# bchess/k8s-1m

Hardware: AMD Instinct MI355X
Metric: pods scheduled/sec at 1M nodes (1/2/4/8 GPU) + % of HBM roofline (higher is better)
Workload: dtype int64+f64

## Files before the change

### k8s-1m_amd/csrc/ksched_host.cpp

```cpp
#include <atomic>
#include <hip/hip_runtime.h>
#include <rccl/rccl.h>

#include <algorithm>
#include <array>
#include <chrono>
#include <cstdarg>
#include <cstdio>
#include <cstdlib>
#include <condition_variable>
#include <cstring>
#include <deque>
#include <functional>
#include <map>
#include <mutex>
#include <set>
#include <thread>
#include <memory>
#include <string>
#include <unordered_map>
#include <unordered_set>
#include <vector>

#include "ksched.h"
// ... 246 lines not shown
  uint32_t dict_version = 0;
  uint32_t names_version = 0;
  bool ext = false, norm = false;
  uint32_t cap_pods = 0;
  size_t cap_words = 0;
  PodDev *d_pods = nullptr;
  double *d_pinv = nullptr;
  uint64_t *d_clauses = nullptr;
  DevResult *d_results = nullptr;
  DevResult *h_results = nullptr;
  PodDev *h_pods = nullptr;
  double *h_pinv = nullptr;
  uint64_t *h_clauses = nullptr;
  size_t n_words = 0;
  bool uploaded = false;
  std::vector<uint32_t> set_ids;
  std::vector<uint8_t> spread;
  bool any_spread = false;
  std::vector<SoloNeeds> solo;
  std::vector<uint64_t> ports;
  std::vector<uint8_t> rep;
  std::vector<uint32_t> class_refs;
  std::vector<uint32_t> term_refs;
  uint64_t *d_cmask = nullptr, *h_cmask = nullptr;
  uint8_t *d_marks = nullptr;
  uint32_t *d_cls = nullptr, *h_cls = nullptr;
  bool dups = false;
  bool ran = false;
  ForgetBits forgotten;
  bool queued = false, done = false;
  ks_status run_status = KS_OK;
  std::string run_err;
};

struct LgPost {
  hipEvent_t ev = nullptr;
  const void *ptr = nullptr;
  std::vector<double> vals;
};
struct LocalGroup : Rendezvous<LgPost> {
  using Post = LgPost;
  explicit LocalGroup(uint32_t n) : Rendezvous<LgPost>(n) {}
};

struct ks_ctx {
  ks_config cfg{};
  std::string err;
  hipStream_t stream = nullptr;
  hipStream_t rstream = nullptr;
  hipStream_t sstream = nullptr;
  hipEvent_t ev_sw[2] = {nullptr, nullptr}, ev_res[2] = {nullptr, nullptr};
  hipEvent_t ev_swept[2] = {nullptr, nullptr}, ev_fixed[2] = {nullptr, nullptr};
  uint32_t *d_flags = nullptr;
  uint32_t round_seq = 0;
  uint32_t seq_of[2] = {0, 0};
  bool value_sync = true;
  uint32_t sync_timeout_ms = 60000;
  std::atomic<bool> wedged{false};
  hipStream_t diag_stream = nullptr;
  uint32_t flag_want[4] = {0, 0, 0, 0};
  uint32_t *h_diag = nullptr;
  int32_t stall_flag = -1;
  uint32_t stall_us = 0;
  ks_fit_strategy fit{KS_FIT_LEAST_ALLOCATED, 1, 1, 0};
  FitParams fit_params{0, 1, 1, fit_weight_rcp(1), fit_weight_rcp(1), fit_weight_rcp(2)};
  uint32_t fit_general = 0;
  std::vector<ks_fit_shape_point> fit_shape;
  std::vector<std::pair<uint32_t, int32_t>> fit_x;
  std::vector<std::string> fit_x_names;
  std::vector<int64_t> ba_list;
  std::vector<std::string> ba_names;
  bool early_fix = true;
  uint32_t resolve_mode = KS_RESOLVE_AUTO;
  uint32_t par_max_passes = 32, serial_rounds = 4;
  bool res_profile = false;
  bool dedup = true;
  bool tuple_guess = true;
  uint32_t timing_every = 8, ext_npl = 2;
  uint32_t sweep_blocks = 4096, sweep_blocks_ext = 16384;
  uint64_t sweep_geom[2][8] = {};
  bool ev_profile = false;
  bool run_profile = false;
  double prof[PROF_SLOTS] = {};
  struct EvProf {
    uint64_t runs = 0, events = 0;
    double s = 0;
  } ev_prof[4];
  uint32_t cap = 0, S = 1, npl = 8, P = 256, K = 256;
  std::vector<Shard> shards;
  uint32_t npos = 0;
  std::vector<uint32_t> slot_pos;
  NodeTable t{};
  NodeTable run_t{};
  Shard *d_shards = nullptr;
  uint32_t *d_slot_pos = nullptr;
  uint32_t *d_start = nullptr;
  uint32_t *h_start = nullptr;
  uint32_t *d_norm = nullptr;
  double *d_norm_inv = nullptr;
  PodStat *d_pstat = nullptr;
  uint32_t *d_fix = nullptr;
  uint32_t *d_dedup = nullptr;
  bool dedup_used[2] = {false, false};
  BlockRec *d_brec = nullptr;
  size_t brec_bytes = 0;
  uint64_t *d_srec = nullptr, *d_frec = nullptr;
// ... 2404 lines not shown
  a.slot_pos = c->d_slot_pos;
  a.w = Weights{c->cfg.weight_fit, c->cfg.weight_balanced, c->cfg.weight_taint, c->cfg.weight_affinity,
                c->cfg.weight_image};
  a.fs = c->fit_params;
  a.fit_general = c->fit_general;
  a.fit_table = c->d_fit_table;
  if ((size_t)nloc * c->P * bmax * sizeof(BlockRec) > c->brec_bytes)
    return c->fail(KS_ERR_INVALID, "block record buffer too small");

  const bool early = b->norm && !multi && c->early_fix;
  a.pstat_sweep = early ? 1u : 0u;
  if (k >= 2) {
    if ((st = hand_wait(c, c->stream, 2, c->ev_res[q], c->seq_of[q]))) return st;
    if (b->norm && !early && (st = hand_wait(c, c->stream, 3, c->ev_fixed[pq], c->seq_of[pq]))) return st;
    HIPC(c, launch_advance_writeback(a, c->d_carry + (size_t)q * MAX_P, c->d_pipe + 4 + q, c->stream));
  } else {
    HIPC(c, launch_advance(a, c->stream));
  }
  hipEvent_t e0 = nullptr, e1 = nullptr;
  if (tm) {
    e0 = get_event(c);
    e1 = get_event(c);
    HIPC(c, hipEventRecord(e0, c->stream));
  }
  if (early) HIPC(c, hipMemsetAsync(c->d_pstat, 0, (size_t)c->P * sizeof(PodStat), c->stream));
  HIPC(c, launch_sweep(a, b->ext, bmax, groups, nloc, c->stream));
  ++c->sweeps_issued;
  {
    uint64_t *g = c->sweep_geom[b->ext ? 1 : 0];
    ++g[0];
    g[1] = knpl;
    g[2] = b->ext ? sweep_label_words(knpl, a.t.lw) : 0;
    g[3] = sub;
    g[4] = bmax;
    g[5] = groups;
    g[6] = pg;
  }
  if (tm) {
    HIPC(c, hipEventRecord(e1, c->stream));
    c->ev_sweep.emplace_back(e0, e1);
  }
  const uint32_t seq = ++c->round_seq;
  c->seq_of[q] = seq;
  hipStream_t ss = c->sstream;
  if (early) {
    HIPC(c, launch_norm_check(a, c->stream));
    RoundArgs f = a;
    f.fix = 1;
    f.pg = MAX_PG;
    HIPC(c, launch_sweep(f, true, bmax, (c->P + MAX_PG - 1) / MAX_PG, nloc, c->stream));
  }
  if ((st = hand_signal(c, c->stream, 0, c->ev_swept[q], seq)) || (st = hand_wait(c, ss, 0, c->ev_swept[q], seq))) return st;
  if (b->norm && !early) HIPC(c, hipMemsetAsync(c->d_pstat, 0, (size_t)c->P * sizeof(PodStat), ss));
  HIPC(c, launch_merge(a, nloc, ss));
  if (b->norm && !early) {
    if (multi && (st = coll_allreduce_max_u32(c, (uint32_t *)c->d_pstat, 4 * (size_t)c->P, ss))) return st;
    HIPC(c, launch_norm_check(a, ss));
    RoundArgs f = a;
    f.fix = 1;
    f.pg = MAX_PG;
    HIPC(c, launch_sweep(f, true, bmax, (c->P + MAX_PG - 1) / MAX_PG, nloc, ss));
    if ((st = hand_signal(c, ss, 3, c->ev_fixed[q], seq))) return st;
    HIPC(c, launch_merge(f, nloc, ss));
  }
  if (multi) {
    const size_t words = (size_t)c->P * RW;
    if ((st = coll_allgather(c, a.srec, words * 8, ss))) return st;
  }
  if (c->S > 1) HIPC(c, launch_merge_shards(a, ss));
  HIPC(c, launch_gather_cand(a, b->ext, ss));
  if (k > 0) {
    if ((st = hand_wait(c, ss, 2, c->ev_res[pq], seq - 1))) return st;
    HIPC(c, launch_patch(a, b->ext, ss));
  }
  if ((st = hand_signal(c, ss, 1, c->ev_sw[q], seq)) || (st = hand_wait(c, c->rstream, 1, c->ev_sw[q], seq))) return st;
  if (tm) {
    e0 = get_event(c);
    e1 = get_event(c);
    HIPC(c, hipEventRecord(e0, c->rstream));
  }
  {
    RoundArgs ra = a;
    ra.flag_res = c->value_sync ? c->d_flags + 2 : nullptr;
    ra.seq = seq;
    ra.stall_us = 0;
    if (c->stall_flag == 2) {
      ra.stall_us = c->stall_us;
      c->stall_flag = -1;
    }
    c->flag_want[2] = seq;
    ra.par_max_passes = c->par_max_passes;
    ra.prof = c->res_profile ? c->d_counters + 16 : nullptr;
    ra.serial_rounds = c->serial_rounds;
    ra.rmode = c->resolve_mode == KS_RESOLVE_AUTO ? c->d_flags + 4 : nullptr;
    ra.serial_only = c->resolve_mode == KS_RESOLVE_SERIAL ? 1u : 0u;
    HIPC(c, launch_resolve(ra, b->ext, c->rstream));
  }
  if (tm) {
    HIPC(c, hipEventRecord(e1, c->rstream));
    c->ev_resolve.emplace_back(e0, e1);
  }
  HIPC(c, hipEventRecord(c->ev_res[q], c->rstream));
  return KS_OK;
}

ks_status drain_rounds(ks_ctx *c, uint32_t rounds, void *h_res, const void *d_res, size_t res_bytes) {
  for (uint32_t k = rounds >= 2 ? rounds - 2 : 0; k < rounds; ++k) {
    const uint32_t q = k & 1u;
    HIPC(c, hipStreamWaitEvent(c->stream, c->ev_res[q], 0));
    HIPC(c, launch_writeback(c->t, c->d_carry + (size_t)q * MAX_P, c->d_pipe + 4 + q, c->stream));
  }
  if (res_bytes) HIPC(c, hipMemcpyAsync(h_res, d_res, res_bytes, hipMemcpyDeviceToHost, c->stream));
  HIPC(c, hipMemcpyAsync(c->h_start, c->d_start, 4, hipMemcpyDeviceToHost, c->stream));
  return sync_bounded(c, c->stream, "a pipeline run's drain");
}


ks_status batch_acquire(ks_ctx *c, uint32_t n, size_t words, ks_batch **out) {
  const uint32_t need = std::max<uint32_t>(n, 1);
  ks_batch *b = nullptr;
  {
    std::lock_guard<std::mutex> g(c->pool_mu);
    size_t bi = SIZE_MAX;
    for (size_t i = 0; i < c->pool.size(); ++i)
      if (c->pool[i]->cap_pods >= need && (bi == SIZE_MAX || c->pool[i]->cap_pods < c->pool[bi]->cap_pods)) bi = i;
    if (bi != SIZE_MAX) {
      b = c->pool[bi];
      c->pool.erase(c->pool.begin() + (long)bi);
// ... 2551 lines not shown
```

### k8s-1m_amd/csrc/ksched_kernels.hip

```cpp
#include <hip/hip_runtime.h>

#include <utility>

#include "ksched_dev.hpp"
#include "ksched_eval.hpp"
#include "ksched_kernels.hpp"
#include "ksched_instr.hpp"
#include "ksched_util.hpp"

namespace ks {




typedef unsigned u32x4 __attribute__((ext_vector_type(4)));
typedef const __attribute__((address_space(4))) u32x4 *const_words;
__device__ __forceinline__ PodDev load_pod_requests(const PodDev *pods, uint32_t i) {
  static_assert(offsetof(PodDev, req_cpu_d) == 32 && offsetof(PodDev, nz100_cpu) == 48 &&
                offsetof(PodDev, tol_hard) == 64, "PodDev: the binary64 request fields");
  const const_words src = (const_words)(pods + i);
  const u32x4 w2 = src[2], w3 = src[3];
  PodDev p = {};
  __builtin_memcpy(&p.req_cpu_d, &w2, 16);
  __builtin_memcpy(&p.nz100_cpu, &w3, 16);
// ... 508 lines not shown
  __syncthreads();
  if (threadIdx.x % WAVE == 0) scratch[wid] = v;
  __syncthreads();
  uint32_t s = 0;
  for (uint32_t i = 0; i < nw; ++i) s += scratch[i];
  __syncthreads();
  return s;
}

__device__ void merge_lists(const uint64_t *keys, size_t list_stride, const uint64_t *bounds,
                            size_t bound_stride, uint32_t nl, uint32_t len, uint32_t K, uint64_t *out,
                            uint64_t *s_sort, uint64_t *s_scr, uint32_t *s_cnt, uint32_t *s_u32) {
  uint64_t b = 0;
  for (uint32_t i = threadIdx.x; i < nl; i += blockDim.x) b = max(b, bounds[i * bound_stride]);
  b = block_max_u64(b, s_scr);
  uint32_t cnt = 0;
  for (uint32_t i = threadIdx.x; i < nl; i += blockDim.x)
    for (uint32_t q = 0; q < len; ++q) cnt += keys[i * list_stride + q] > b;
  cnt = block_sum_u32(cnt, s_u32);
  if (cnt > MERGE_CAP) {
    const uint32_t c = MERGE_CAP / nl;
    uint64_t b2 = b;
    for (uint32_t i = threadIdx.x; i < nl; i += blockDim.x)
      if (c < len) b2 = max(b2, keys[i * list_stride + c]);
    b = block_max_u64(b2, s_scr);
  }
  if (threadIdx.x == 0) *s_cnt = 0;
  __syncthreads();
  for (uint32_t i = threadIdx.x; i < nl; i += blockDim.x)
    for (uint32_t q = 0; q < len; ++q) {
      const uint64_t k = keys[i * list_stride + q];
      if (k > b) {
        const uint32_t at = atomicAdd(s_cnt, 1u);
        if (at < MERGE_CAP) s_sort[at] = k;
      }
    }
  __syncthreads();
  const uint32_t n = min(*s_cnt, (uint32_t)MERGE_CAP);
  uint32_t m = 64;
  while (m < n) m <<= 1;
  for (uint32_t i = n + threadIdx.x; i < m; i += blockDim.x) s_sort[i] = 0;
  __syncthreads();
  bitonic_desc(s_sort, m);
  const uint32_t keep = min(n, K);
  if (n > K) b = max(b, s_sort[K]);
  for (uint32_t i = threadIdx.x; i < K; i += blockDim.x) out[REC_HDR_WORDS + i] = i < keep ? s_sort[i] : 0ull;
  if (threadIdx.x == 0) {
    out[0] = b;
    ((uint32_t *)out)[2] = keep;
  }
}

constexpr int MERGE_THREADS = 1024;
__global__ __launch_bounds__(MERGE_THREADS) void merge_kernel(RoundArgs a) {
  __shared__ uint64_t s_sort[MERGE_CAP];
  __shared__ uint64_t s_scr[16];
  __shared__ uint32_t s_u32[16];
  __shared__ uint32_t s_cnt;
  __shared__ uint32_t s_wc[MERGE_THREADS / WAVE][NFILT + 5];
  const uint32_t start = uniform_u32(*a.sstart);
  const uint32_t r = blockIdx.x;
  if (start + r >= a.npods || r >= a.P) return;
  if (a.fix && a.fix_flag[r] == 0) return;
  if (a.rep != nullptr && a.rep[r] != r) return;
  const uint32_t sh = blockIdx.y;
  const Shard s = a.shards[a.shard0 + sh];
  const uint32_t nb = (s.waves * a.sub + 3) / 4;
  const BlockRec *br = a.brec + ((size_t)sh * a.P + r) * a.bstride;
  uint64_t *out = a.srec + ((size_t)(a.shard0 + sh) * a.P + r) * rec_words(a.K);
  merge_lists(&br[0].keys[0], sizeof(BlockRec) / 8, &br[0].bound, sizeof(BlockRec) / 8, nb, BLOCK_KEYS, a.K,
              out, s_sort, s_scr, &s_cnt, s_u32);
  int32_t c[NFILT + 3];
  for (int q = 0; q < NFILT + 3; ++q) c[q] = 0;
  uint32_t tmx = 0, nmx = 0;
  for (uint32_t i = threadIdx.x; i < nb; i += blockDim.x) {
    c[0] += br[i].feasible;
    for (int q = 0; q < NFILT; ++q) c[1 + q] += br[i].fails[q];
    c[6] += br[i].tt_cnt;
    c[7] += br[i].na_cnt;
    tmx = max(tmx, br[i].tt_max);
    nmx = max(nmx, br[i].na_max);
  }
  const uint32_t wid = threadIdx.x / WAVE;
#pragma unroll
  for (int q = 0; q < NFILT + 3; ++q) c[q] = wave_sum_i32_dpp(c[q]);
  tmx = wave_max_u32_dpp(tmx);
  nmx = wave_max_u32_dpp(nmx);
  if (threadIdx.x % WAVE == 0) {
    for (int q = 0; q < NFILT + 3; ++q) s_wc[wid][q] = (uint32_t)c[q];
    s_wc[wid][NFILT + 3] = tmx;
    s_wc[wid][NFILT + 4] = nmx;
  }
  __syncthreads();
  if (threadIdx.x == 0) {
    uint32_t t[NFILT + 5] = {};
    for (uint32_t w = 0; w < blockDim.x / WAVE; ++w) {
      for (int q = 0; q < NFILT + 3; ++q) t[q] += s_wc[w][q];
      t[NFILT + 3] = max(t[NFILT + 3], s_wc[w][NFILT + 3]);
      t[NFILT + 4] = max(t[NFILT + 4], s_wc[w][NFILT + 4]);
    }
    ShardRecHdr *h = (ShardRecHdr *)out;
    h->feasible = t[0];
    for (int q = 0; q < NFILT; ++q) h->fails[q] = t[1 + q];
    h->tt_cnt = t[6];
    h->na_cnt = t[7];
    if (a.pstat != nullptr && !a.fix && !a.pstat_sweep) {
      PodStat *ps = a.pstat + r;
      if (t[NFILT + 3]) atomicMax(&ps->tt_max, t[NFILT + 3]);
      if (t[NFILT + 4]) atomicMax(&ps->na_max, t[NFILT + 4]);
      if (t[0]) atomicMax(&ps->any_feasible, 1u);
    }
  }
}


__global__ __launch_bounds__(MAX_P) void norm_check_kernel(RoundArgs a) {
  __shared__ uint32_t s_wn[MAX_P / WAVE];
  const uint32_t start = uniform_u32(*a.sstart);
  const uint32_t r = threadIdx.x;
  bool wrong = false, listed = false;
  if (r < a.P && start + r < a.npods) {
    const PodDev &p = a.pods[start + r];
    const uint32_t rr = a.rep != nullptr ? a.rep[r] : r;
    PodStat st = a.pstat[rr];
    if (a.pstat_sweep) {
      st.any_feasible = st.tt_max != 0u;
      st.tt_max = st.tt_max ? st.tt_max - 1u : 0u;
      st.na_max = st.na_max ? st.na_max - 1u : 0u;
    }
    uint32_t tt = p.tt_guess, na = p.na_guess;
    if (st.any_feasible) {
      wrong = ((p.flags & PF_TT) && st.tt_max != tt) || ((p.flags & PF_NA) && st.na_max != na);
      tt = st.tt_max;
      na = st.na_max;
    }
    a.norm_max[2 * r] = tt;
    a.norm_max[2 * r + 1] = na;
    a.norm_inv[2 * r] = tt ? 1.0 / (double)tt : 0.0;
    a.norm_inv[2 * r + 1] = na ? 1.0 / (double)na : 0.0;
    a.fix_flag[r] = wrong ? 1u : 0u;
    if (wrong) mark_pod(a.marks, start + r, MARK_FIX);
    listed = wrong && rr == r;
  }
  const uint64_t wb = __ballot(listed);
  const uint32_t nw = (uint32_t)__popcll(wb), nwrong = (uint32_t)__popcll(__ballot(wrong));
  const uint32_t wid = threadIdx.x / WAVE, lane = threadIdx.x % WAVE;
  if (lane == 0) s_wn[wid] = nw;
  if (nwrong && lane == 0) atomicAdd((unsigned long long *)&a.counters[4], (unsigned long long)nwrong);
  __syncthreads();
  uint32_t idx = (uint32_t)__popcll(wb & ((1ull << lane) - 1ull)), total = 0;
#pragma unroll
  for (int w = 0; w < MAX_P / WAVE; ++w) {
    idx += (uint32_t)w < wid ? s_wn[w] : 0u;
    total += s_wn[w];
  }
  if (listed) a.fix_list[idx] = r;
  if (r >= total) a.fix_list[r] = FIX_NONE;
  if (r < MAX_P / MAX_PG) a.fix_group[r] = r * MAX_PG < total ? 1u : 0u;
}

__global__ __launch_bounds__(256) void merge_shards_kernel(RoundArgs a) {
  __shared__ uint64_t s_sort[MERGE_CAP];
  __shared__ uint64_t s_scr[16];
  __shared__ uint32_t s_u32[16];
  __shared__ uint32_t s_cnt;
  const uint32_t start = uniform_u32(*a.sstart);
  const uint32_t r = blockIdx.x;
  if (start + r >= a.npods || r >= a.P) return;
  if (a.rep != nullptr && a.rep[r] != r) return;
  const uint32_t W = rec_words(a.K);
  const uint64_t *in = a.srec + (size_t)r * W;
  const size_t stride = (size_t)a.P * W;
  uint64_t *out = a.frec + (size_t)r * W;
  merge_lists(in + REC_HDR_WORDS, stride, in, stride, a.total_shards, a.K, a.K, out, s_sort, s_scr, &s_cnt, s_u32);
  if (threadIdx.x == 0) {
    ShardRecHdr *h = (ShardRecHdr *)out;
    uint32_t f = 0, ttc = 0, nac = 0, fl[NFILT] = {0, 0, 0, 0, 0};
    for (uint32_t q = 0; q < a.total_shards; ++q) {
      const ShardRecHdr *x = (const ShardRecHdr *)(in + q * stride);
      f += x->feasible;
      ttc += x->tt_cnt;
      nac += x->na_cnt;
      for (int z = 0; z < NFILT; ++z) fl[z] += x->fails[z];
    }
    h->feasible = f;
    h->tt_cnt = ttc;
    h->na_cnt = nac;
    for (int z = 0; z < NFILT; ++z) h->fails[z] = fl[z];
  }
}

__device__ __forceinline__ CandRow cand_row(int64_t acpu, int64_t amem, int64_t rc, int64_t rm, int64_t zc, int64_t zm,
                                            int32_t apods, int32_t np, uint32_t pos) {
  CandRow w;
  w.acpu = (double)acpu;
  w.amem = (double)amem;
  w.inv_cpu = acpu ? 1.0 / w.acpu : 0.0;
  w.inv_mem = amem ? 1.0 / w.amem : 0.0;
  w.rc = (double)rc;
  w.rm = (double)rm;
  w.zc100 = (double)zc * 100.0;
  w.zm100 = (double)zm * 100.0;
  w.apods = apods;
  w.np = np;
  w.pos = pos;
  w._pad = 0;
  return w;
}

template <bool EXT>
__global__ __launch_bounds__(256) void gather_cand_kernel(RoundArgs a) {
  const uint32_t start = uniform_u32(*a.sstart);
  const uint32_t r = blockIdx.x;
  if (start + r >= a.npods || r >= a.P) return;
  if (a.rep != nullptr && a.rep[r] != r) return;
  const uint64_t *rec = a.frec + (size_t)r * rec_words(a.K);
  const uint32_t nk = ((const ShardRecHdr *)rec)->nkeys;
  for (uint32_t t = threadIdx.x; t < nk; t += blockDim.x) {
    const uint64_t k = rec[REC_HDR_WORDS + t];
    const uint32_t pos = a.slot_pos[0xFFFFFFFFu - (uint32_t)k];
    a.crow[(size_t)r * a.K + t] = cand_row(a.t.acpu[pos], a.t.amem[pos], a.t.rcpu[pos], a.t.rmem[pos], a.t.zcpu[pos],
                                           a.t.zmem[pos], a.t.apods[pos], a.t.npods[pos], pos);
    if (EXT) {
      CandExt x;
      x.w[0] = a.t.hard[pos];
      x.w[1] = a.t.prefer[pos];
#pragma unroll
      for (int q = 0; q < LW; ++q) x.w[2 + q] = a.t.lab[(size_t)q * a.t.npos + pos];
#pragma unroll
      for (int q = 0; q < NNUM; ++q) x.w[2 + LW + q] = (uint64_t)a.t.num[(size_t)q * a.t.npos + pos];
      a.cext[(size_t)r * a.K + t] = x;
    }
  }
}

constexpr int PHASH = 1024;
static_assert(2 * MAX_P >= MAX_K, "patch thread counts");


__device__ __forceinline__ uint32_t count_greater(const uint64_t *v, uint32_t n, uint64_t x) {
  uint32_t lo = 0, hi = n;
  while (lo < hi) {
    const uint32_t mid = (lo + hi) >> 1;
    if (v[mid] > x) lo = mid + 1;
    else hi = mid;
  }
  return lo;
}


template <bool EXT, int PATCH_THREADS, int GF = 0>
__global__ __launch_bounds__(PATCH_THREADS) void patch_kernel(RoundArgs a) {
  static_assert(PATCH_THREADS >= MAX_P, "one thread per carried node");
  constexpr int NW = PATCH_THREADS / WAVE;
  __shared__ uint32_t s_hkey[PHASH];
  __shared__ uint64_t s_k1[MAX_P];
  __shared__ uint64_t s_ckey[MAX_P];
  __shared__ uint64_t s_lkey[MAX_K];
  __shared__ uint32_t s_wl[NW], s_wc[NW];
  __shared__ int32_t s_wd[NW][NFILT + 3];
  __shared__ uint64_t s_wdrop[NW];

  const uint32_t tid = threadIdx.x, lane = tid % WAVE, wid = tid / WAVE;
  const uint32_t start = uniform_u32(*a.act);
  const uint32_t r = blockIdx.x;
  if (a.first || start >= a.npods || uniform_u32(*a.sstart) != start || start + r >= a.npods) return;
  if (a.rep != nullptr && uniform_u32(a.rep[r]) != r) return;
  const uint32_t nc = uniform_u32(*a.carry_in_n);
  if (nc == 0) return;
  const PodDev p = a.pods[start + r];
  uint64_t *rec = a.frec + (size_t)r * rec_words(a.K);
  ShardRecHdr *hdr = (ShardRecHdr *)rec;
  const uint64_t bound = hdr->bound;
  const uint32_t nk = hdr->nkeys;
  int64_t tt_max = 0, na_max = 0;
  if (EXT) {
    tt_max = a.norm_max[2 * r];
    na_max = a.norm_max[2 * r + 1];
  }
  for (uint32_t i = tid; i < PHASH; i += PATCH_THREADS) s_hkey[i] = 0;
  if constexpr (GF == 2) fit_table_stage(a.fit_table);
  __syncthreads();

  int32_t d[NFILT + 3] = {0, 0, 0, 0, 0, 0, 0, 0};
  uint64_t k1 = 0;
  if (tid < nc) {
    const CarryRec &cr = a.carry_in[tid];
    NodeExt ce{};
    if (EXT) ext_from_words(cr.ext, ce);
    const double inv_cpu = cr.acpu ? 1.0 / (double)cr.acpu : 0.0, inv_mem = cr.amem ? 1.0 / (double)cr.amem : 0.0;
    const NodeRegs r1 = make_regs_inv(cr.acpu, cr.amem, cr.rc, cr.rm, cr.zc, cr.zm, cr.apods, cr.np, cr.slot,
                                      inv_cpu, inv_mem);
    NodeRegs r0 = r1;
    r0.free_cpu = (double)(cr.acpu - cr.rc0);
    r0.free_mem = (double)(cr.amem - cr.rm0);
    r0.bits = (r1.bits & ~2u) | ((int64_t)cr.np0 + 1 <= (int64_t)cr.apods ? 2u : 0u);
    const int st0 = filter<EXT>(p, a.clauses, r0, ce);
    const int st1 = filter<EXT>(p, a.clauses, r1, ce);
    if (st1 == ST_FEASIBLE) k1 = pack_key(total_score<EXT, GF>(p, a.clauses, r1, ce, a.w, a.fs, tt_max, na_max), cr.slot);
    if (st0 != st1) status_delta<EXT>(p, a.clauses, st0, st1, ce, cr.slot, tt_max, na_max, d);
    uint32_t h = rhash(cr.slot);
    while (atomicCAS(&s_hkey[h], 0u, cr.slot + 1) != 0u) h = (h + 1) & (PHASH - 1);
  }
  if (tid < MAX_P) s_k1[tid] = k1;
  if (__ballot(d[0] | d[1] | d[2] | d[3] | d[4] | d[5] | d[6] | d[7]) != 0) {
// ... 383 lines not shown
    } else {
      sweep_kernel<8, true, 4, GF><<<g, SWEEP_THREADS, 0, st>>>(a);
    }
  } else {
    if (a.npl == 2) sweep_kernel<2, false, LW, GF><<<g, SWEEP_THREADS, 0, st>>>(a);
    else if (a.npl == 4) sweep_kernel<4, false, LW, GF><<<g, SWEEP_THREADS, 0, st>>>(a);
    else sweep_kernel<8, false, LW, GF><<<g, SWEEP_THREADS, 0, st>>>(a);
  }
  return hipGetLastError();
}

hipError_t launch_sweep(const RoundArgs &a, bool ext, uint32_t nblocks, uint32_t ngroups, uint32_t nshards,
                        hipStream_t st) {
  dim3 g(nblocks, ngroups, nshards);
  if (a.fit_general == 2) return launch_sweep_fit<2>(a, ext, g, st);
  if (a.fit_general) return launch_sweep_fit<1>(a, ext, g, st);
  if (ext) {
    const uint32_t lwu = sweep_label_words(a.npl, a.t.lw);
    if (a.npl == 2) {
      if (lwu == 1) sweep_kernel<2, true, 1><<<g, SWEEP_THREADS, 0, st>>>(a);
      else if (lwu == 2) sweep_kernel<2, true, 2><<<g, SWEEP_THREADS, 0, st>>>(a);
      else sweep_kernel<2, true, 4><<<g, SWEEP_THREADS, 0, st>>>(a);
    } else if (a.npl == 4) {
      if (lwu == 1) sweep_kernel<4, true, 1><<<g, SWEEP_THREADS, 0, st>>>(a);
      else if (lwu == 2) sweep_kernel<4, true, 2><<<g, SWEEP_THREADS, 0, st>>>(a);
      else sweep_kernel<4, true, 4><<<g, SWEEP_THREADS, 0, st>>>(a);
    } else {
      sweep_kernel<8, true, 4><<<g, SWEEP_THREADS, 0, st>>>(a);
    }
  } else {
    if (a.npl == 2) sweep_kernel<2, false><<<g, SWEEP_THREADS, 0, st>>>(a);
    else if (a.npl == 4) sweep_kernel<4, false><<<g, SWEEP_THREADS, 0, st>>>(a);
    else sweep_kernel<8, false><<<g, SWEEP_THREADS, 0, st>>>(a);
  }
  return hipGetLastError();
}

hipError_t launch_merge(const RoundArgs &a, uint32_t nshards, hipStream_t st) {
  merge_kernel<<<dim3(a.P, nshards), MERGE_THREADS, 0, st>>>(a);
  return hipGetLastError();
}

hipError_t launch_merge_shards(const RoundArgs &a, hipStream_t st) {
  merge_shards_kernel<<<dim3(a.P), 256, 0, st>>>(a);
  return hipGetLastError();
}

hipError_t launch_gather_cand(const RoundArgs &a, bool ext, hipStream_t st) {
  if (ext) gather_cand_kernel<true><<<a.P, 256, 0, st>>>(a);
  else gather_cand_kernel<false><<<a.P, 256, 0, st>>>(a);
  return hipGetLastError();
}

hipError_t launch_advance(const RoundArgs &a, hipStream_t st) {
  advance_kernel<<<1, ADV_THREADS, 0, st>>>(a);
  return hipGetLastError();
}

hipError_t launch_advance_writeback(const RoundArgs &a, const CarryRec *carry, const uint32_t *n, hipStream_t st) {
  advance_writeback_kernel<<<2, ADV_THREADS, 0, st>>>(a, a.t, carry, n);
  return hipGetLastError();
}

hipError_t launch_writeback(const NodeTable &t, const CarryRec *carry, const uint32_t *n, hipStream_t st) {
  writeback_kernel<<<2, 256, 0, st>>>(t, carry, n);
  return hipGetLastError();
}

template <int GF>
static hipError_t launch_patch_fit(const RoundArgs &a, bool ext, hipStream_t st) {
  if (a.K <= (uint32_t)MAX_P) {
    if (ext) patch_kernel<true, MAX_P, GF><<<a.P, MAX_P, 0, st>>>(a);
    else patch_kernel<false, MAX_P, GF><<<a.P, MAX_P, 0, st>>>(a);
  } else {
    if (ext) patch_kernel<true, MAX_K, GF><<<a.P, MAX_K, 0, st>>>(a);
    else patch_kernel<false, MAX_K, GF><<<a.P, MAX_K, 0, st>>>(a);
  }
  return hipGetLastError();
}

hipError_t launch_patch(const RoundArgs &a, bool ext, hipStream_t st) {
  if (a.fit_general == 2) return launch_patch_fit<2>(a, ext, st);
  if (a.fit_general) return launch_patch_fit<1>(a, ext, st);
  if (a.K <= (uint32_t)MAX_P) {
    if (ext) patch_kernel<true, MAX_P><<<a.P, MAX_P, 0, st>>>(a);
    else patch_kernel<false, MAX_P><<<a.P, MAX_P, 0, st>>>(a);
  } else {
    if (ext) patch_kernel<true, MAX_K><<<a.P, MAX_K, 0, st>>>(a);
    else patch_kernel<false, MAX_K><<<a.P, MAX_K, 0, st>>>(a);
  }
  return hipGetLastError();
}

hipError_t launch_scatter_rows(const NodeTable &t, const uint32_t *pos, const int64_t *core, const uint64_t *ext,
                               uint32_t n, uint32_t flags, hipStream_t st) {
  if (!n) return hipSuccess;
  scatter_rows_kernel<<<(n + 255) / 256, 256, 0, st>>>(t, pos, core, ext, n, flags);
  return hipGetLastError();
}

hipError_t launch_apply_deltas(const NodeTable &t, const uint32_t *pos, const int64_t *delta, uint32_t n,
                               hipStream_t st) {
  if (!n) return hipSuccess;
  apply_deltas_kernel<<<(n + 255) / 256, 256, 0, st>>>(t, pos, delta, n);
  return hipGetLastError();
}
// ... 32 lines not shown
```

### k8s-1m_amd/csrc/ksched_kernels.hpp

```cpp
#pragma once

#include <hip/hip_runtime.h>

#include "ksched_dev.hpp"

namespace ks {

constexpr int MAX_PG = 64;
constexpr int MAX_P = 256;
constexpr int MAX_K = 512;
constexpr uint32_t FIX_NONE = 0xFFFFFFFFu;
constexpr int CTR_CPU_SHARED = 9;
constexpr int CTR_PAR_PASSES = 12, CTR_PAR_ROUNDS = 13, CTR_PAR_BAILS = 14, CTR_PAR_ONESTEP = 15;
constexpr uint8_t MARK_FIX = 1;
constexpr uint8_t MARK_ROUND_START = 2;
constexpr uint8_t MARK_AFTER_WASTE = 4;

struct RoundArgs {
  NodeTable t;
  const Shard *shards;
  uint32_t total_shards;
  uint32_t shard0;
  uint32_t npl;
  uint32_t sub;
  uint32_t P;
  uint32_t pg;
  uint32_t K;
  uint32_t npods;
  uint32_t bstride;
  uint32_t evaluated;
  uint32_t lnpl;
  const PodDev *pods;
  const uint64_t *clauses;
  uint32_t *d_start;
  uint32_t *sstart;
  const uint32_t *prev_sstart;
  uint32_t *act;
  uint32_t *act_next;
  const uint32_t *prev_act;
  const CarryRec *carry_in;
  const uint32_t *carry_in_n;
  CarryRec *carry_out;
  uint32_t *carry_out_n;
  uint32_t first;
  uint32_t *norm_max;
  double *norm_inv;
  const double *guess_inv;
  PodStat *pstat;
  uint32_t *fix_flag;
  uint32_t *fix_group;
  uint32_t *fix_list;
  uint32_t fix;
  uint32_t pstat_sweep;
  uint32_t *flag_res;
  uint32_t seq;
  uint32_t stall_us;
  uint32_t *rmode;
  uint32_t par_max_passes, serial_rounds;
  uint32_t serial_only;
  uint64_t *prof;
  uint8_t *marks;
  const uint32_t *cls;
  uint32_t *rep, *ulist, *nuniq;
  uint32_t sort_cpu;
  BlockRec *brec;
  uint64_t *srec;
  uint64_t *frec;
  void *results;
  CandRow *crow;
  CandExt *cext;
  const uint32_t *slot_pos;
  uint64_t *counters;
  Weights w;
  FitParams fs;
  uint32_t fit_general;
  const uint32_t *fit_table;
};

struct DumpArgs {
  NodeTable t;
  const uint32_t *slot_pos;
  uint32_t nslots;
  const PodDev *pods;
  const uint64_t *clauses;
  uint32_t *norm_max;
  int32_t *out;
  Weights w;
  FitParams fs;
  uint32_t fit_general;
  const uint32_t *fit_table;
};

constexpr uint32_t SLOT_NONE = 0xFFFFFFFFu;
constexpr int SPREAD_DUMP_WORDS = 14;
enum SpreadLaunch : uint32_t {
  SPL_PREP = 1u,
  SPL_MIN = 2u,
  SPL_SCORE = 4u,
  SPL_AFF = 8u,
  SPL_XFIT = 16u,
  SPL_BAL = 32u,
  SPL_PORTS = 64u,
};
struct SpreadArgs {
  NodeTable t;
  const uint32_t *pos_slot;
  const uint32_t *slot_pos;
  uint32_t npos;
  uint32_t pod;
  const PodDev *pods;
  const uint64_t *clauses;
  const uint64_t *cmask;
  const uint32_t *dom;
  uint32_t *cnt;
  int64_t *xalloc, *xreq;
  uint32_t *dcnt;
  uint32_t *dflag;
  uint32_t *tcnt;
  uint32_t *adcnt;
  int64_t *ipa_raw;
  uint32_t dom_cap;
  uint32_t ndom[MAX_TOPO_KEYS];
  SpreadAcc *acc;
  int8_t *st;
  int64_t *raw;
  uint64_t *part;
  DevResult *results;
  int32_t *dump;
  uint32_t no_commit;
// ... 56 lines not shown
constexpr int DPB_STAGE = 2048;
constexpr int DPB_MAX_BLOCKS = 512;
struct DiagPair {
  uint32_t pod, slot;
};
struct DiagPodsArgs {
  NodeTable t;
  const uint32_t *pos_slot;
  uint32_t npos;
  uint32_t first, count;
  const PodDev *pods;
  const uint64_t *clauses;
  DiagRec *recs;
  DiagPair *list;
  unsigned long long *list_n;
  uint32_t list_cap;
};
hipError_t launch_diagnose_pods(const DiagPodsArgs &a, bool ext, hipStream_t st);
uint32_t diagnose_pods_blocks(uint32_t npos);
hipError_t launch_spread_front(const SpreadArgs &a, uint32_t passes, hipStream_t st);
struct TopkBest;
struct ExplainOut;
struct ExplainArgs {
  uint64_t *blk_keys;
  TopkBest *blk_best;
  uint64_t *keys;
  ExplainOut *out;
  uint32_t k;
};
hipError_t launch_explain(const SpreadArgs &a, const ExplainArgs &x, uint32_t passes, hipStream_t st);
hipError_t launch_replica_run(const SpreadArgs &a, const ReplicaArgs &r, void *sort_tmp, size_t sort_tmp_bytes,
                              uint32_t passes, hipStream_t st);
hipError_t launch_sort_pairs(const uint64_t *kin, uint64_t *kout, const uint64_t *vin, uint64_t *vout, uint32_t n,
                             uint32_t end_bit, void *tmp, size_t *tmp_bytes, hipStream_t st);
hipError_t launch_class_commit(const DevResult *res, const uint64_t *cmask, const uint32_t *slot_pos, uint32_t *cnt,
                               uint32_t npos, uint32_t lo, uint32_t hi, hipStream_t st);
hipError_t launch_scatter_u32(uint32_t *col, const uint64_t *idx, const uint32_t *val, uint32_t n, hipStream_t st);
hipError_t launch_add_u32(uint32_t *col, const uint64_t *idx, const int32_t *delta, uint32_t n, hipStream_t st);
hipError_t launch_umax_u32(uint32_t *dst, const uint32_t *src, uint32_t n, hipStream_t st);
hipError_t launch_scatter_i64(int64_t *col, const uint64_t *idx, const int64_t *val, uint32_t n, bool add,
                              hipStream_t st);
hipError_t launch_ports_update(uint64_t *col, const uint32_t *pos, const uint64_t *bits, uint32_t n, bool clear,
                               hipStream_t st);

hipError_t launch_norm_check(const RoundArgs &a, hipStream_t st);
inline uint32_t sweep_label_words(uint32_t knpl, uint32_t lw) {
  return knpl == 8 ? 4u : lw <= 1 ? 1u : lw <= 2 ? 2u : 4u;
}
hipError_t launch_sweep(const RoundArgs &a, bool ext, uint32_t nblocks, uint32_t ngroups, uint32_t nshards,
                        hipStream_t st);
hipError_t launch_merge(const RoundArgs &a, uint32_t nshards, hipStream_t st);
hipError_t launch_merge_shards(const RoundArgs &a, hipStream_t st);
hipError_t launch_gather_cand(const RoundArgs &a, bool ext, hipStream_t st);
hipError_t launch_patch(const RoundArgs &a, bool ext, hipStream_t st);
hipError_t launch_resolve(const RoundArgs &a, bool ext, hipStream_t st);
hipError_t launch_advance(const RoundArgs &a, hipStream_t st);
hipError_t launch_advance_writeback(const RoundArgs &a, const CarryRec *carry, const uint32_t *n, hipStream_t st);
hipError_t launch_writeback(const NodeTable &t, const CarryRec *carry, const uint32_t *n, hipStream_t st);
hipError_t launch_scatter_rows(const NodeTable &t, const uint32_t *pos, const int64_t *core, const uint64_t *ext,
                               uint32_t n, uint32_t flags, hipStream_t st);
hipError_t launch_apply_deltas(const NodeTable &t, const uint32_t *pos, const int64_t *delta, uint32_t n,
                               hipStream_t st);
hipError_t launch_gather_rows(const NodeTable &t, const uint32_t *pos, int64_t *out, uint32_t n, hipStream_t st);
hipError_t launch_scatter_u64(uint64_t *col, const uint32_t *pos, const uint64_t *val, uint32_t n,
                              hipStream_t st);
hipError_t launch_dump(const DumpArgs &a, hipStream_t st);
struct ForgetArgs {
  NodeTable t;
  const uint32_t *slot_pos;
  const DevResult *results;
  const PodDev *pods;
  const uint64_t *clauses;
  const uint32_t *idx;
  int64_t *xreq;
  uint64_t *used_ports;
  uint32_t *missed;
  uint64_t n_words;
  uint32_t n, npods, nslots;
};
constexpr uint32_t FORGET_THREADS = 256;
hipError_t launch_forget(const ForgetArgs &a, hipStream_t st);
hipError_t launch_stall(uint32_t usec, hipStream_t st);

}
```

### k8s-1m_amd/csrc/ksched_util.hpp

```cpp
#pragma once

#include <hip/hip_runtime.h>

#include <utility>

#include "ksched_dev.hpp"
#include "ksched_eval.hpp"

namespace ks {

constexpr int KS_PLUGIN_FIT_IDX = 4;
typedef __attribute__((address_space(1))) void gvoid_t;
typedef __attribute__((address_space(3))) void lvoid_t;

template <class F, int... I>
__device__ __forceinline__ void static_for_impl(F &&f, std::integer_sequence<int, I...>) {
  (f(std::integral_constant<int, I>{}), ...);
}
template <int N, class F>
__device__ __forceinline__ void static_for(F &&f) {
  static_for_impl(f, std::make_integer_sequence<int, N>{});
}

__device__ __forceinline__ uint64_t wave_max_u64(uint64_t v) {
// ... 77 lines not shown
  v = max(v, dpp32<0xB1>(v));
  v = max(v, dpp32<0x4E>(v));
  v = max(v, dpp32<0x141>(v));
  v = max(v, dpp32<0x140>(v));
  return smax_u32(smax_u32((uint32_t)__builtin_amdgcn_readlane((int)v, 0), (uint32_t)__builtin_amdgcn_readlane((int)v, 16)),
                  smax_u32((uint32_t)__builtin_amdgcn_readlane((int)v, 32), (uint32_t)__builtin_amdgcn_readlane((int)v, 48)));
}
__device__ __forceinline__ uint32_t writelane_u32(uint32_t v, uint32_t x, uint32_t l) {
#pragma clang diagnostic push
#pragma clang diagnostic ignored "-Winline-asm"
  asm("s_mov_b32 m0, %2\n\tv_writelane_b32 %0, %1, m0" : "+v"(v) : "s"(x), "s"(l) : "m0");
#pragma clang diagnostic pop
  return v;
}
__device__ __forceinline__ void wave_lds_order() {
  __builtin_amdgcn_fence(__ATOMIC_RELEASE, "wavefront");
  __builtin_amdgcn_wave_barrier();
  __builtin_amdgcn_fence(__ATOMIC_ACQUIRE, "wavefront");
}
__device__ __forceinline__ WaveTuple tuple_ror8(const WaveTuple &w) {
  return {dpp32<0x128>(w.t1), dpp32<0x128>(w.t2), dpp32<0x128>(w.t3), dpp32<0x128>(w.B)};
}
__device__ __forceinline__ WaveTuple tuple_xor(const WaveTuple &w, int m) {
  return {(uint32_t)__shfl_xor((int)w.t1, m, WAVE), (uint32_t)__shfl_xor((int)w.t2, m, WAVE),
          (uint32_t)__shfl_xor((int)w.t3, m, WAVE), (uint32_t)__shfl_xor((int)w.B, m, WAVE)};
}
__device__ __forceinline__ uint32_t min8_u32(uint32_t v) {
  v = min(v, dpp32<0xB1>(v));
  v = min(v, dpp32<0x4E>(v));
  return min(v, dpp32<0x141>(v));
}
__device__ __forceinline__ int32_t sum8_i32(int32_t v) {
  v += (int32_t)dpp32<0xB1>((uint32_t)v);
  v += (int32_t)dpp32<0x4E>((uint32_t)v);
  return v + (int32_t)dpp32<0x141>((uint32_t)v);
}
__device__ __forceinline__ int32_t wave_sum_i32_dpp(int32_t v) {
  v = sum8_i32(v);
  v += (int32_t)dpp32<0x140>((uint32_t)v);
  return __builtin_amdgcn_readlane(v, 0) + __builtin_amdgcn_readlane(v, 16) + __builtin_amdgcn_readlane(v, 32) +
         __builtin_amdgcn_readlane(v, 48);
}

__device__ __forceinline__ void stall_for(uint32_t usec) {
  const uint64_t t0 = __builtin_amdgcn_s_memrealtime();
  while (__builtin_amdgcn_s_memrealtime() - t0 < 100ull * usec) __builtin_amdgcn_s_sleep(127);
}

__device__ __forceinline__ void signal_done(uint32_t *flag, uint32_t seq, uint32_t stall_us = 0) {
  if (flag == nullptr) return;
  if (stall_us) stall_for(stall_us);
  __threadfence_system();
  __hip_atomic_store(flag, seq, __ATOMIC_RELEASE, __HIP_MEMORY_SCOPE_SYSTEM);
}

__device__ __forceinline__ void mark_pod(uint8_t *marks, uint32_t i, uint8_t bit) {
  atomicOr((uint32_t *)(marks + (i & ~3u)), (uint32_t)bit << (8u * (i & 3u)));
}

__device__ __forceinline__ uint32_t rhash(uint32_t x) { return (x * 2654435761u) >> 22; }

struct alignas(16) RNode {
  CandRow row;
  double rc0, rm0;
  int32_t np0;
  uint32_t slot;
  uint32_t _pad[2];
};
static_assert(sizeof(RNode) == 112, "RNode layout");

__device__ __forceinline__ RNode rnode_from_row(const CandRow &w, uint32_t slot) {
  RNode n;
  n.row = w;
  n.rc0 = w.rc;
  n.rm0 = w.rm;
  n.np0 = w.np;
  n.slot = slot;
  n._pad[0] = n._pad[1] = 0;
  return n;
}

__device__ __forceinline__ void rnode_add(RNode &n, const PodDev &p) {
  n.row.rc += p.req_cpu_d;
  n.row.rm += p.req_mem_d;
  n.row.zc100 += p.nz100_cpu;
  n.row.zm100 += p.nz100_mem;
  n.row.np += 1;
}

__device__ __forceinline__ NodeRegs rnode_regs(const RNode &n, double rc, double rm, int32_t np) {
  const CandRow &w = n.row;
  NodeRegs r;
  r.slot = n.slot;
  r.free_cpu = w.acpu - rc;
  r.free_mem = w.amem - rm;
  r.rcpu = rc;
  r.rmem = rm;
  r.lf100_cpu = w.acpu * 100.0 - w.zc100;
  r.lf100_mem = w.amem * 100.0 - w.zm100;
  r.acpu_d = w.acpu;
  r.amem_d = w.amem;
  r.inv_cpu = w.inv_cpu;
  r.inv_mem = w.inv_mem;
  const bool ac = w.acpu != 0.0, am = w.amem != 0.0;
  r.bamul = (ac && am) ? 0.5 : 0.0;
  r.lashift = (ac && am) ? 1u : 0u;
// ... 32 lines not shown
```

Baseline: 948,400.

## Fuse merge with candidate gather and signal handoff from patch kernel

On single-shard, single-GPU runs, the merge and gather_cand kernels become one kernel. When there are few enough block records, it loads each BlockRec as five 16-byte vectors, one per thread, filters keys against the block maximum bound, sorts them, and gathers candidate rows straight from shared memory. Separately, the patch kernel now raises the cross-stream handoff flag itself through a last-block atomic counter, replacing a separate hand_signal. The goal is fewer kernel launches and a shorter round-trip on the critical path, in exchange for more code paths and a per-round counter whose target must stay in step with the number of patch blocks.

```diff
diff --git a/k8s-1m_amd/csrc/ksched_host.cpp b/k8s-1m_amd/csrc/ksched_host.cpp
--- a/k8s-1m_amd/csrc/ksched_host.cpp
+++ b/k8s-1m_amd/csrc/ksched_host.cpp
@@ -322,6 +322,7 @@
   hipEvent_t ev_sw[2] = {nullptr, nullptr}, ev_res[2] = {nullptr, nullptr};
   hipEvent_t ev_swept[2] = {nullptr, nullptr}, ev_fixed[2] = {nullptr, nullptr};
   uint32_t *d_flags = nullptr;
+  uint32_t patch_blocks = 0;
   uint32_t round_seq = 0;
   uint32_t seq_of[2] = {0, 0};
   bool value_sync = true;
@@ -2832,7 +2833,9 @@
   }
   if ((st = hand_signal(c, c->stream, 0, c->ev_swept[q], seq)) || (st = hand_wait(c, ss, 0, c->ev_swept[q], seq))) return st;
   if (b->norm && !early) HIPC(c, hipMemsetAsync(c->d_pstat, 0, (size_t)c->P * sizeof(PodStat), ss));
-  HIPC(c, launch_merge(a, nloc, ss));
+  const bool fused = c->S == 1 && !multi;
+  if (fused) HIPC(c, launch_merge_gather(a, b->ext, ss));
+  else HIPC(c, launch_merge(a, nloc, ss));
   if (b->norm && !early) {
     if (multi && (st = coll_allreduce_max_u32(c, (uint32_t *)c->d_pstat, 4 * (size_t)c->P, ss))) return st;
     HIPC(c, launch_norm_check(a, ss));
@@ -2841,19 +2844,36 @@
     f.pg = MAX_PG;
     HIPC(c, launch_sweep(f, true, bmax, (c->P + MAX_PG - 1) / MAX_PG, nloc, ss));
     if ((st = hand_signal(c, ss, 3, c->ev_fixed[q], seq))) return st;
-    HIPC(c, launch_merge(f, nloc, ss));
+    if (fused) HIPC(c, launch_merge_gather(f, b->ext, ss));
+    else HIPC(c, launch_merge(f, nloc, ss));
   }
   if (multi) {
     const size_t words = (size_t)c->P * RW;
     if ((st = coll_allgather(c, a.srec, words * 8, ss))) return st;
   }
   if (c->S > 1) HIPC(c, launch_merge_shards(a, ss));
-  HIPC(c, launch_gather_cand(a, b->ext, ss));
-  if (k > 0) {
+  if (!fused) HIPC(c, launch_gather_cand(a, b->ext, ss));
+  if (k > 0 && c->value_sync) {
     if ((st = hand_wait(c, ss, 2, c->ev_res[pq], seq - 1))) return st;
-    HIPC(c, launch_patch(a, b->ext, ss));
-  }
-  if ((st = hand_signal(c, ss, 1, c->ev_sw[q], seq)) || (st = hand_wait(c, c->rstream, 1, c->ev_sw[q], seq))) return st;
+    RoundArgs pa = a;
+    pa.flag_done = c->d_flags + 1;
+    pa.done_count = c->d_flags + 7;
+    pa.done_target = c->patch_blocks += a.P;
+    pa.seq = seq;
+    if (c->stall_flag == 1) {
+      pa.stall_us = c->stall_us;
+      c->stall_flag = -1;
+    }
+    c->flag_want[1] = seq;
+    HIPC(c, launch_patch(pa, b->ext, ss));
+  } else {
+    if (k > 0) {
+      if ((st = hand_wait(c, ss, 2, c->ev_res[pq], seq - 1))) return st;
+      HIPC(c, launch_patch(a, b->ext, ss));
+    }
+    if ((st = hand_signal(c, ss, 1, c->ev_sw[q], seq))) return st;
+  }
+  if ((st = hand_wait(c, c->rstream, 1, c->ev_sw[q], seq))) return st;
   if (tm) {
     e0 = get_event(c);
     e1 = get_event(c);
diff --git a/k8s-1m_amd/csrc/ksched_kernels.hip b/k8s-1m_amd/csrc/ksched_kernels.hip
--- a/k8s-1m_amd/csrc/ksched_kernels.hip
+++ b/k8s-1m_amd/csrc/ksched_kernels.hip
@@ -584,6 +584,54 @@
 }
 
 constexpr int MERGE_THREADS = 1024;
+__device__ __forceinline__ void merge_block_counts(const BlockRec *br, uint32_t nb, int32_t (&c)[NFILT + 3],
+                                                   uint32_t &tmx, uint32_t &nmx) {
+  for (int q = 0; q < NFILT + 3; ++q) c[q] = 0;
+  tmx = 0, nmx = 0;
+  for (uint32_t i = threadIdx.x; i < nb; i += blockDim.x) {
+    c[0] += br[i].feasible;
+    for (int q = 0; q < NFILT; ++q) c[1 + q] += br[i].fails[q];
+    c[6] += br[i].tt_cnt;
+    c[7] += br[i].na_cnt;
+    tmx = max(tmx, br[i].tt_max);
+    nmx = max(nmx, br[i].na_max);
+  }
+}
+
+__device__ __forceinline__ void merge_counts(const RoundArgs &a, uint32_t r, uint64_t *out, int32_t (&c)[NFILT + 3],
+                                             uint32_t tmx, uint32_t nmx, uint32_t (*s_wc)[NFILT + 5]) {
+  const uint32_t wid = threadIdx.x / WAVE;
+#pragma unroll
+  for (int q = 0; q < NFILT + 3; ++q) c[q] = wave_sum_i32_dpp(c[q]);
+  tmx = wave_max_u32_dpp(tmx);
+  nmx = wave_max_u32_dpp(nmx);
+  if (threadIdx.x % WAVE == 0) {
+    for (int q = 0; q < NFILT + 3; ++q) s_wc[wid][q] = (uint32_t)c[q];
+    s_wc[wid][NFILT + 3] = tmx;
+    s_wc[wid][NFILT + 4] = nmx;
+  }
+  __syncthreads();
+  if (threadIdx.x == 0) {
+    uint32_t t[NFILT + 5] = {};
+    for (uint32_t w = 0; w < blockDim.x / WAVE; ++w) {
+      for (int q = 0; q < NFILT + 3; ++q) t[q] += s_wc[w][q];
+      t[NFILT + 3] = max(t[NFILT + 3], s_wc[w][NFILT + 3]);
+      t[NFILT + 4] = max(t[NFILT + 4], s_wc[w][NFILT + 4]);
+    }
+    ShardRecHdr *h = (ShardRecHdr *)out;
+    h->feasible = t[0];
+    for (int q = 0; q < NFILT; ++q) h->fails[q] = t[1 + q];
+    h->tt_cnt = t[6];
+    h->na_cnt = t[7];
+    if (a.pstat != nullptr && !a.fix && !a.pstat_sweep) {
+      PodStat *ps = a.pstat + r;
+      if (t[NFILT + 3]) atomicMax(&ps->tt_max, t[NFILT + 3]);
+      if (t[NFILT + 4]) atomicMax(&ps->na_max, t[NFILT + 4]);
+      if (t[0]) atomicMax(&ps->any_feasible, 1u);
+    }
+  }
+}
+
 __global__ __launch_bounds__(MERGE_THREADS) void merge_kernel(RoundArgs a) {
   __shared__ uint64_t s_sort[MERGE_CAP];
   __shared__ uint64_t s_scr[16];
@@ -603,46 +651,9 @@
   merge_lists(&br[0].keys[0], sizeof(BlockRec) / 8, &br[0].bound, sizeof(BlockRec) / 8, nb, BLOCK_KEYS, a.K,
               out, s_sort, s_scr, &s_cnt, s_u32);
   int32_t c[NFILT + 3];
-  for (int q = 0; q < NFILT + 3; ++q) c[q] = 0;
-  uint32_t tmx = 0, nmx = 0;
-  for (uint32_t i = threadIdx.x; i < nb; i += blockDim.x) {
-    c[0] += br[i].feasible;
-    for (int q = 0; q < NFILT; ++q) c[1 + q] += br[i].fails[q];
-    c[6] += br[i].tt_cnt;
-    c[7] += br[i].na_cnt;
-    tmx = max(tmx, br[i].tt_max);
-    nmx = max(nmx, br[i].na_max);
-  }
-  const uint32_t wid = threadIdx.x / WAVE;
-#pragma unroll
-  for (int q = 0; q < NFILT + 3; ++q) c[q] = wave_sum_i32_dpp(c[q]);
-  tmx = wave_max_u32_dpp(tmx);
-  nmx = wave_max_u32_dpp(nmx);
-  if (threadIdx.x % WAVE == 0) {
-    for (int q = 0; q < NFILT + 3; ++q) s_wc[wid][q] = (uint32_t)c[q];
-    s_wc[wid][NFILT + 3] = tmx;
-    s_wc[wid][NFILT + 4] = nmx;
-  }
-  __syncthreads();
-  if (threadIdx.x == 0) {
-    uint32_t t[NFILT + 5] = {};
-    for (uint32_t w = 0; w < blockDim.x / WAVE; ++w) {
-      for (int q = 0; q < NFILT + 3; ++q) t[q] += s_wc[w][q];
-      t[NFILT + 3] = max(t[NFILT + 3], s_wc[w][NFILT + 3]);
-      t[NFILT + 4] = max(t[NFILT + 4], s_wc[w][NFILT + 4]);
-    }
-    ShardRecHdr *h = (ShardRecHdr *)out;
-    h->feasible = t[0];
-    for (int q = 0; q < NFILT; ++q) h->fails[q] = t[1 + q];
-    h->tt_cnt = t[6];
-    h->na_cnt = t[7];
-    if (a.pstat != nullptr && !a.fix && !a.pstat_sweep) {
-      PodStat *ps = a.pstat + r;
-      if (t[NFILT + 3]) atomicMax(&ps->tt_max, t[NFILT + 3]);
-      if (t[NFILT + 4]) atomicMax(&ps->na_max, t[NFILT + 4]);
-      if (t[0]) atomicMax(&ps->any_feasible, 1u);
-    }
-  }
+  uint32_t tmx, nmx;
+  merge_block_counts(br, nb, c, tmx, nmx);
+  merge_counts(a, r, out, c, tmx, nmx, s_wc);
 }
 
 
@@ -741,15 +752,9 @@
 }
 
 template <bool EXT>
-__global__ __launch_bounds__(256) void gather_cand_kernel(RoundArgs a) {
-  const uint32_t start = uniform_u32(*a.sstart);
-  const uint32_t r = blockIdx.x;
-  if (start + r >= a.npods || r >= a.P) return;
-  if (a.rep != nullptr && a.rep[r] != r) return;
-  const uint64_t *rec = a.frec + (size_t)r * rec_words(a.K);
-  const uint32_t nk = ((const ShardRecHdr *)rec)->nkeys;
+__device__ __forceinline__ void gather_rows(const RoundArgs &a, uint32_t r, const uint64_t *keys, uint32_t nk) {
   for (uint32_t t = threadIdx.x; t < nk; t += blockDim.x) {
-    const uint64_t k = rec[REC_HDR_WORDS + t];
+    const uint64_t k = keys[t];
     const uint32_t pos = a.slot_pos[0xFFFFFFFFu - (uint32_t)k];
     a.crow[(size_t)r * a.K + t] = cand_row(a.t.acpu[pos], a.t.amem[pos], a.t.rcpu[pos], a.t.rmem[pos], a.t.zcpu[pos],
                                            a.t.zmem[pos], a.t.apods[pos], a.t.npods[pos], pos);
@@ -766,6 +771,84 @@
   }
 }
 
+template <bool EXT>
+__global__ __launch_bounds__(256) void gather_cand_kernel(RoundArgs a) {
+  const uint32_t start = uniform_u32(*a.sstart);
+  const uint32_t r = blockIdx.x;
+  if (start + r >= a.npods || r >= a.P) return;
+  if (a.rep != nullptr && a.rep[r] != r) return;
+  const uint64_t *rec = a.frec + (size_t)r * rec_words(a.K);
+  gather_rows<EXT>(a, r, rec + REC_HDR_WORDS, ((const ShardRecHdr *)rec)->nkeys);
+}
+
+template <bool EXT>
+__global__ __launch_bounds__(MERGE_THREADS) void merge_gather_kernel(RoundArgs a) {
+  static_assert(MERGE_THREADS * BLOCK_KEYS <= MERGE_CAP, "one record per thread stays under the cap");
+  static_assert(BLOCK_KEYS == 4 && NFILT == 5 && sizeof(BlockRec) == 80, "BlockRec as five 16-byte pieces");
+  __shared__ uint64_t s_sort[MERGE_CAP];
+  __shared__ uint64_t s_scr[16];
+  __shared__ uint32_t s_u32[16];
+  __shared__ uint32_t s_cnt;
+  __shared__ uint32_t s_wc[MERGE_THREADS / WAVE][NFILT + 5];
+  const uint32_t start = uniform_u32(*a.sstart);
+  const uint32_t r = blockIdx.x;
+  if (start + r >= a.npods || r >= a.P) return;
+  if (a.fix && a.fix_flag[r] == 0) return;
+  if (a.rep != nullptr && a.rep[r] != r) return;
+  const Shard s = a.shards[a.shard0];
+  const uint32_t nb = (s.waves * a.sub + 3) / 4;
+  const BlockRec *br = a.brec + (size_t)r * a.bstride;
+  uint64_t *out = a.srec + ((size_t)a.shard0 * a.P + r) * rec_words(a.K);
+  int32_t c[NFILT + 3];
+  uint32_t tmx, nmx;
+  if (nb > (uint32_t)MERGE_THREADS) {
+    merge_lists(&br[0].keys[0], sizeof(BlockRec) / 8, &br[0].bound, sizeof(BlockRec) / 8, nb, BLOCK_KEYS, a.K,
+                out, s_sort, s_scr, &s_cnt, s_u32);
+    merge_block_counts(br, nb, c, tmx, nmx);
+  } else {
+    uint4 v0{}, v1{}, v2{}, v3{}, v4{};
+    if (threadIdx.x < nb) {
+      const uint4 *p = (const uint4 *)(br + threadIdx.x);
+      v0 = p[0], v1 = p[1], v2 = p[2], v3 = p[3], v4 = p[4];
+    }
+    const uint64_t k0 = (uint64_t)v0.y << 32 | v0.x, k1 = (uint64_t)v0.w << 32 | v0.z;
+    const uint64_t k2 = (uint64_t)v1.y << 32 | v1.x, k3 = (uint64_t)v1.w << 32 | v1.z;
+    uint64_t b = block_max_u64((uint64_t)v2.y << 32 | v2.x, s_scr);
+    if (threadIdx.x == 0) s_cnt = 0;
+    __syncthreads();
+    const uint32_t mine = (uint32_t)(k0 > b) + (uint32_t)(k1 > b) + (uint32_t)(k2 > b) + (uint32_t)(k3 > b);
+    if (mine) {
+      uint32_t at = atomicAdd(&s_cnt, mine);
+      if (k0 > b) s_sort[at++] = k0;
+      if (k1 > b) s_sort[at++] = k1;
+      if (k2 > b) s_sort[at++] = k2;
+      if (k3 > b) s_sort[at++] = k3;
+    }
+    __syncthreads();
+    const uint32_t n = s_cnt;
+    uint32_t m = 64;
+    while (m < n) m <<= 1;
+    for (uint32_t i = n + threadIdx.x; i < m; i += blockDim.x) s_sort[i] = 0;
+    __syncthreads();
+    bitonic_desc(s_sort, m);
+    const uint32_t keep = min(n, a.K);
+    if (n > a.K) b = max(b, s_sort[a.K]);
+    for (uint32_t i = threadIdx.x; i < a.K; i += blockDim.x) out[REC_HDR_WORDS + i] = i < keep ? s_sort[i] : 0ull;
+    if (threadIdx.x == 0) {
+      out[0] = b;
+      ((uint32_t *)out)[2] = keep;
+    }
+    c[0] = (int32_t)v2.z;
+    c[1] = (int32_t)v2.w, c[2] = (int32_t)v3.x, c[3] = (int32_t)v3.y, c[4] = (int32_t)v3.z, c[5] = (int32_t)v3.w;
+    c[6] = (int32_t)v4.x;
+    c[7] = (int32_t)v4.y;
+    tmx = v4.z;
+    nmx = v4.w;
+  }
+  merge_counts(a, r, out, c, tmx, nmx, s_wc);
+  gather_rows<EXT>(a, r, s_sort, min(min(s_cnt, (uint32_t)MERGE_CAP), a.K));
+}
+
 constexpr int PHASH = 1024;
 static_assert(2 * MAX_P >= MAX_K, "patch thread counts");
 
@@ -781,8 +864,17 @@
 }
 
 
+template <bool EXT, int PATCH_THREADS, int GF>
+__device__ __forceinline__ void patch_block(const RoundArgs &a);
+
 template <bool EXT, int PATCH_THREADS, int GF = 0>
 __global__ __launch_bounds__(PATCH_THREADS) void patch_kernel(RoundArgs a) {
+  patch_block<EXT, PATCH_THREADS, GF>(a);
+  signal_when_all_done(a.flag_done, a.done_count, a.done_target, a.seq, a.stall_us);
+}
+
+template <bool EXT, int PATCH_THREADS, int GF>
+__device__ __forceinline__ void patch_block(const RoundArgs &a) {
   static_assert(PATCH_THREADS >= MAX_P, "one thread per carried node");
   constexpr int NW = PATCH_THREADS / WAVE;
   __shared__ uint32_t s_hkey[PHASH];
@@ -1272,6 +1364,12 @@
   return hipGetLastError();
 }
 
+hipError_t launch_merge_gather(const RoundArgs &a, bool ext, hipStream_t st) {
+  if (ext) merge_gather_kernel<true><<<a.P, MERGE_THREADS, 0, st>>>(a);
+  else merge_gather_kernel<false><<<a.P, MERGE_THREADS, 0, st>>>(a);
+  return hipGetLastError();
+}
+
 hipError_t launch_advance(const RoundArgs &a, hipStream_t st) {
   advance_kernel<<<1, ADV_THREADS, 0, st>>>(a);
   return hipGetLastError();
diff --git a/k8s-1m_amd/csrc/ksched_kernels.hpp b/k8s-1m_amd/csrc/ksched_kernels.hpp
--- a/k8s-1m_amd/csrc/ksched_kernels.hpp
+++ b/k8s-1m_amd/csrc/ksched_kernels.hpp
@@ -75,6 +75,9 @@
   FitParams fs;
   uint32_t fit_general;
   const uint32_t *fit_table;
+  uint32_t *flag_done;
+  uint32_t *done_count;
+  uint32_t done_target;
 };
 
 struct DumpArgs {
@@ -237,6 +240,7 @@
 hipError_t launch_merge(const RoundArgs &a, uint32_t nshards, hipStream_t st);
 hipError_t launch_merge_shards(const RoundArgs &a, hipStream_t st);
 hipError_t launch_gather_cand(const RoundArgs &a, bool ext, hipStream_t st);
+hipError_t launch_merge_gather(const RoundArgs &a, bool ext, hipStream_t st);
 hipError_t launch_patch(const RoundArgs &a, bool ext, hipStream_t st);
 hipError_t launch_resolve(const RoundArgs &a, bool ext, hipStream_t st);
 hipError_t launch_advance(const RoundArgs &a, hipStream_t st);
diff --git a/k8s-1m_amd/csrc/ksched_util.hpp b/k8s-1m_amd/csrc/ksched_util.hpp
--- a/k8s-1m_amd/csrc/ksched_util.hpp
+++ b/k8s-1m_amd/csrc/ksched_util.hpp
@@ -153,6 +153,17 @@
   if (stall_us) stall_for(stall_us);
   __threadfence_system();
   __hip_atomic_store(flag, seq, __ATOMIC_RELEASE, __HIP_MEMORY_SCOPE_SYSTEM);
+}
+
+__device__ __forceinline__ void signal_when_all_done(uint32_t *flag, uint32_t *count, uint32_t target, uint32_t seq,
+                                                     uint32_t stall_us) {
+  if (flag == nullptr) return;
+  __threadfence();
+  __syncthreads();
+  if (threadIdx.x == 0) {
+    const uint32_t before = __hip_atomic_fetch_add(count, 1u, __ATOMIC_ACQ_REL, __HIP_MEMORY_SCOPE_AGENT);
+    if (before + 1u == target) signal_done(flag, seq, stall_us);
+  }
 }
 
 __device__ __forceinline__ void mark_pod(uint8_t *marks, uint32_t i, uint8_t bit) {
```

Result: slower. 896,400 (-5.5%).
